# facebookresearch/rela

Hardware: AMD Instinct MI355X
Metric: env-steps/s (Ape-X Atari 84x84x4, actor tick + learner grad-step) (higher is better)
Workload: dtype f32 (f32 operands as 3 exact bf16 parts on bf16 MFMA; f32-accurate); 1 GPU; Ape-X DQN 80x80 envs/GPU, actor+learner on one MI355X, replay 2^20, B=512, A=18, n=3; device-resident static frames; parallelism=single

## Files before the change

### include/rela_amd.h

```cpp
#ifndef RELA_AMD_H
#define RELA_AMD_H

#include <stdint.h>

#ifdef __cplusplus
extern "C" {
#endif

#define RELA_OK 0
#define RELA_EINVAL (-1)
#define RELA_ENODEV (-2)
#define RELA_ENOMEM (-3)
#define RELA_ESTATE (-4)
#define RELA_ESCAN (-5)
#define RELA_EWOULDBLOCK (-6)

const char* rela_last_error(void);
int rela_abi_version(void);

int rela_stream_create(void** out, int device);
void rela_stream_destroy(void* stream, int device);
int rela_stream_synchronize(void* stream, int device);
int rela_stream_wait_stream(void* waiter, void* signaler, int device);
int rela_memcpy_h2d_async(void* dst_dev, const void* src_host, int64_t bytes, void* stream, int device);
// ... 129 lines not shown
                                  void* stream);
int rela_ffnet_debug_fc_stamps(const rela_ffnet* net, int n, const uint8_t* a3_records, unsigned long long* out_host,
                               void* stream);
int64_t rela_ffnet_workspace_bytes(const rela_ffnet* net, int n);
enum { RELA_WS_NOT_WRITTEN = 0, RELA_WS_F32 = 1, RELA_WS_SPLIT_BF16 = 2, RELA_WS_SPLIT3 = 3 };
typedef struct {
  int64_t a1, a2, a3, h, ha, gx, fc_part, rec2, rec3;
  int32_t precision, trunk, fc, fc_slices, fc_per;
  int32_t a1_format, a2_format, a3_format;
  int32_t a3_records, x_in_gx;
} rela_debug_workspace_view;
int rela_ffnet_debug_workspace(const rela_ffnet* net, int n, rela_debug_workspace_view* view);
int rela_ffnet_debug_forward_store_frames(const rela_ffnet* net, int n, const uint8_t* s_dev, const float* legal_dev,
                                          float* q_dev, void* workspace_dev, int64_t workspace_bytes, void* rows_dev,
                                          int first, int ring, int* copied, void* stream);

int rela_ffnet_forward(const rela_ffnet* net, int n, const uint8_t* s_dev, const float* legal_dev,
                       float* q_dev, void* workspace_dev, int64_t workspace_bytes, void* stream);

int rela_apex_act_from_q(int n, int num_action, int group_rows, const float* q_dev,
                         const float* legal_dev, const float* eps_dev, uint64_t rng_seed,
                         uint64_t rng_offset, int64_t* action_dev, void* stream);

int rela_apex_td_from_q(int n, int num_action, int group_rows, const float* q_dev,
                        const float* q_next_online_dev,
                        const float* q_next_target_dev, const float* next_legal_dev,
                        const int64_t* action_dev, const float* reward_dev,
                        const float* bootstrap_dev, float gamma_n, float* td_err_dev,
                        float* priority_dev, void* stream);

// ... 267 lines not shown
```

### rela_amd/_capi.py

```python
import ctypes as C
import os

import torch

PKG = os.path.dirname(os.path.abspath(__file__))
LIB_PATH = os.path.join(PKG, "librela_amd.so")

if not os.path.exists(LIB_PATH):
    raise ImportError(
        "rela_amd: %s is missing -- the HIP extension has not been built (python -m rela_amd.build). "
        "There is no CPU fallback for this path." % LIB_PATH)

lib = C.CDLL(LIB_PATH)

OK, EINVAL, ENODEV, ENOMEM, ESTATE, ESCAN, EWOULDBLOCK = 0, -1, -2, -3, -4, -5, -6

vp, i32, i64, u64, f32, f64 = C.c_void_p, C.c_int, C.c_int64, C.c_uint64, C.c_float, C.c_double
P = C.POINTER


class ReplayState(C.Structure):
    _fields_ = [("head", C.c_int32), ("tail", C.c_int32), ("size", C.c_int32), ("safe_size", C.c_int32),
                ("ring", C.c_int32), ("n_sampled", C.c_int32), ("num_add", C.c_int64), ("sum", C.c_double),
                ("dev_error", C.c_int32), ("pad", C.c_int32)]
# ... 143 lines not shown
_sig("rela_ffnet_num_action", i32, [vp])
_sig("rela_ffnet_version", C.c_uint64, [vp])
_sig("rela_ffnet_set_precision", i32, [vp, i32])
_sig("rela_ffnet_precision", i32, [vp])
_sig("rela_ffnet_debug_conv12_stamps", i32, [vp, i32, vp, vp, vp])
_sig("rela_ffnet_debug_fc_stamps", i32, [vp, i32, vp, vp, vp])
_sig("rela_ffnet_debug_conv3_stamps", i32, [vp, i32, vp, vp, vp])
_sig("rela_ffnet_debug_conv12_records", i32, [vp, i32, vp, vp, vp, vp, vp, vp])
_sig("rela_ffnet_debug_layout", i32, [vp, i32, P(C.c_char_p), P(i64), P(i32), vp])
_sig("rela_lstmnet_debug_layout", i32, [vp, i32, P(C.c_char_p), P(i64), P(i32), vp])
_sig("rela_lstmnet_set_precision", i32, [vp, i32])
_sig("rela_lstmnet_precision", i32, [vp])
_sig("rela_ffnet_workspace_bytes", i64, [vp, i32])
_sig("rela_ffnet_debug_workspace", i32, [vp, i32, P(DebugWorkspaceView)])
_sig("rela_ffnet_debug_forward_store_frames", i32, [vp, i32, vp, vp, vp, vp, i64, vp, i32, i32, P(i32), vp])
_sig("rela_lstmnet_debug_workspace", i32, [vp, i32, P(DebugWorkspaceView)])
_sig("rela_ffnet_forward", i32, [vp, i32, vp, vp, vp, vp, i64, vp])
_sig("rela_lstmnet_create", i32, [P(vp), i32, i32])
_sig("rela_lstmnet_destroy", None, [vp])
_sig("rela_lstmnet_load", i32, [vp, P(LSTMNetParams), i32, vp])
_sig("rela_lstmnet_num_action", i32, [vp])
_sig("rela_lstmnet_version", C.c_uint64, [vp])
_sig("rela_lstmnet_workspace_bytes", i64, [vp, i32])
_sig("rela_lstmnet_step", i32, [vp, i32, vp, vp, vp, vp, vp, vp, vp, vp, vp, i64, vp])
_sig("rela_apex_act_from_q", i32, [i32, i32, i32, vp, vp, vp, u64, u64, vp, vp])
_sig("rela_apex_td_from_q", i32, [i32, i32, i32, vp, vp, vp, vp, vp, vp, vp, f32, vp, vp, vp])
_sig("rela_apex_actor_create", i32, [P(vp), i32, i32, i32, i32, f32, vp, u64, i32])
_sig("rela_apex_actor_destroy", None, [vp])
_sig("rela_apex_actor_obs_slot", vp, [vp])
_sig("rela_apex_actor_plane_stage", vp, [vp])
# ... 122 lines not shown
```

### rela_amd/csrc/actor.hip

```cpp
#include <cmath>

#include "actor_shard.h"
#include "ffnet_layout.h"

using namespace rela_amd;

struct rela_apex_actor : ActorShardBase {
  float gamma = 0.f, gamma_n = 0.f;
  uint64_t seed = 0;
  float* prio = nullptr;
  void* ws = nullptr;
  int64_t ws_bytes = 0;
  int64_t key_tick = -1;
};

namespace {
constexpr int kTickWin = 64;
}

extern "C" int rela_apex_actor_create(rela_apex_actor** out, int rows, int group_rows, int num_action, int multi_step,
                                      float gamma, rela_replay* replay, uint64_t seed, int device) {
  RELA_CHECK(out && rows >= 1 && group_rows >= 1 && rows % group_rows == 0 && num_action >= 1 && num_action <= 31 &&
                 multi_step >= 1,
             RELA_EINVAL, "rela_apex_actor_create: bad arguments (rows=%d group=%d A=%d n=%d)", rows, group_rows,
// ... 38 lines not shown
extern "C" int rela_apex_actor_set_screen_input(rela_apex_actor* a, int height, int width) {
  return shard_set_screen_input(a, height, width, 3, "rela_apex_actor_set_screen_input");
}
extern "C" int rela_apex_actor_set_screen_input_indexed(rela_apex_actor* a, int height, int width) {
  return shard_set_screen_input(a, height, width, 1, "rela_apex_actor_set_screen_input_indexed");
}
extern "C" void* rela_apex_actor_palette_stage(rela_apex_actor* a) { return a ? a->palettes : nullptr; }
extern "C" void* rela_apex_actor_screen_stage(rela_apex_actor* a) { return a ? a->screens : nullptr; }
extern "C" int rela_apex_actor_screens_to_stacks(rela_apex_actor* a, const uint8_t* restart_host, void* stream_) {
  return shard_screens_to_stacks(a, restart_host, (hipStream_t)stream_, "rela_apex_actor_screens_to_stacks");
}
extern "C" int rela_apex_actor_set_reuse(rela_apex_actor* a, int on) {
  return shard_set_reuse(a, on, "rela_apex_actor_set_reuse");
}
extern "C" int rela_apex_actor_set_fused_insert(rela_apex_actor* a, int on) {
  RELA_CHECK(a && (on == 0 || on == 1), RELA_EINVAL, "rela_apex_actor_set_fused_insert: 0 (off) or 1 (on)");
  a->fused_insert = on != 0;
  return RELA_OK;
}
extern "C" int rela_apex_actor_set_value_rescale(rela_apex_actor* a, float eps) {
  return shard_set_value_rescale(a, eps, "rela_apex_actor_set_value_rescale");
}
extern "C" int rela_apex_actor_set_dedup(rela_apex_actor* a, int units_per_stack) {
  const int rc = shard_set_dedup_common(a, units_per_stack, 0, "rela_apex_actor_set_dedup");
  if (rc == RELA_OK) a->tick_seq.assign(kTickWin, 0);
  return rc;
}
extern "C" float* rela_apex_actor_eps_dev(rela_apex_actor* a) { return a ? a->eps : nullptr; }
extern "C" float* rela_apex_actor_legal_dev(rela_apex_actor* a) { return a ? a->legal : nullptr; }
extern "C" int64_t rela_apex_actor_num_act(const rela_apex_actor* a) { return a ? a->num_act.load() : 0; }
extern "C" const float* rela_apex_actor_last_q_dev(const rela_apex_actor* a) {
  return a ? a->q_hist + (size_t)(a->q_slot < 0 ? 0 : a->q_slot) * a->R * a->A : nullptr;
// ... 96 lines not shown
  if (a->fused_insert && a->dd_ups == 0 && piece == a->R && ffnet_forward_stores_frames(target, a->R)) {
    rc = rela_replay_begin_add(a->replay, a->R, nonblocking, &fused_slot);
    if (rc == RELA_EWOULDBLOCK) fused_slot = -1;
    else if (rc != RELA_OK) return rc;
  }
  if (fused_slot >= 0) {
    void* base = nullptr;
    int rows_ring = 0;
    int64_t row_bytes = 0;
    rc = rela_replay_direct_rows(a->replay, fused_slot, a->R, 1, &base, &rows_ring, &row_bytes, s);
    if (rc == RELA_OK && row_bytes != kObs) {
      set_last_error("rela_apex_actor_post_step: the replay's next_obs rows have %lld bytes, a frame stack %lld",
                     (long long)row_bytes, (long long)kObs);
      rc = RELA_EINVAL;
    }
    if (rc == RELA_OK)
      rc = ffnet_forward_store_frames(target, a->R, obs_n, legal_n, a->q + 3 * QA, a->ws, a->ws_bytes, s,
                                      FrameRows{static_cast<uint8_t*>(base), fused_slot, rows_ring}, &fused_copied);
  } else {
    rc = rela_ffnet_forward(target, a->R, obs_n, legal_n, a->q + 3 * QA, a->ws, a->ws_bytes, s);
  }
  const int64_t* act_t = a->act + (size_t)first * a->R;
  if (rc == RELA_OK)
    rc = td_from_q(a->R, a->A, a->K, q_online_t, q_online_n, a->q + 3 * QA, legal_n, act_t, a->out_r, a->out_b, a->gamma_n,
                   a->vr_eps, nullptr, a->prio, s);
  if (rc != RELA_OK) {
    if (fused_slot >= 0) (void)rela_replay_abort_add(a->replay, fused_slot, a->R);
    return rc;
  }
  const void* rows[10] = {obs_t, obs_n, eps_t, eps_n, legal_t, legal_n, act_t, a->out_r, a->out_t, a->out_b};
  if (a->dd_ups > 0) {
    rows[0] = a->ref_hist + (size_t)first * a->R * a->dd_ups;
    rows[1] = a->ref_hist + (size_t)last * a->R * a->dd_ups;
  }
  const int64_t stack_rb = a->dd_ups > 0 ? (int64_t)sizeof(int32_t) * a->dd_ups : kObs;
  const int64_t rb[10] = {stack_rb, stack_rb, 4, 4, 4 * a->A, 4 * a->A, 8, 4, 1, 4};
  int dropped = dd_drop ? 1 : 0;
  for (int off = 0; off < a->R && !dd_drop; off += piece) {
    const int cnt = a->R - off < piece ? a->R - off : piece;
    const void* prow[10];
    for (int f = 0; f < 10; ++f) prow[f] = static_cast<const uint8_t*>(rows[f]) + (int64_t)off * rb[f];
    int slot = fused_slot;
    if (fused_slot >= 0) {
      if (fused_copied) prow[1] = nullptr;
    } else {
      rc = rela_replay_begin_add(a->replay, cnt, nonblocking, &slot);
      if (rc == RELA_EWOULDBLOCK) {
        dropped = 1;
        continue;
      }
      if (rc != RELA_OK) break;
    }
    if (a->dd_ups > 0) (void)rela_replay_set_block_min_unit(a->replay, slot, cnt, dd_min_seq);
    rc = rela_replay_write_rows(a->replay, slot, 0, cnt, prow, s);
    if (rc == RELA_OK) rc = rela_replay_commit_add_grouped(a->replay, slot, cnt, a->K, a->prio + off, s);
    if (rc != RELA_OK) {
      (void)rela_replay_abort_add(a->replay, slot, cnt);
      break;
    }
// ... 8 lines not shown
```

### rela_amd/csrc/actor_shard.h

```cpp
#pragma once
#include <atomic>
#include <vector>

#include "common.h"
#include "dedup_refs.h"

namespace rela_amd {

constexpr int64_t kObs = 4 * 84 * 84;
constexpr int64_t kPlane = 84 * 84;

struct ActorShardBase {
  int device = 0;
  int R = 0, K = 0, A = 0, n = 0;
  rela_replay* replay = nullptr;
  uint64_t act_calls = 0;
  std::atomic<int64_t> num_act{0};
  int head = 0, count = 0, cur = -1;
  uint8_t* obs = nullptr;
  int64_t* act = nullptr;
  float* rew = nullptr;
  uint8_t* term = nullptr;
  float* eps = nullptr;
  float* legal = nullptr;
  float* eps_hist = nullptr;
  float* legal_hist = nullptr;
  float* q = nullptr;
  float* q_hist = nullptr;
  float *out_r = nullptr, *out_b = nullptr;
  uint8_t* out_t = nullptr;
  std::vector<const void*> qh_net;
  std::vector<uint64_t> qh_version;
  int q_slot = -1;
  int reuse_mode = 1;
  bool fused_insert = true;
  float vr_eps = 0.f;
  uint8_t* restart = nullptr;
  uint8_t* fresh_planes = nullptr;
  uint8_t* screens = nullptr;
  uint8_t* palettes = nullptr;
  uint8_t* screen_prev = nullptr;
  int scr_h = 0, scr_w = 0;
  int dd_ups = 0;
  int64_t dd_cap = 0;
  int32_t* ref_hist = nullptr;
  std::vector<uint8_t> refs_valid;
  std::vector<int64_t> tick_seq;
  int64_t tick = 0;
};

// ... 210 lines not shown
```

### rela_amd/csrc/conv12_s3.h

```cpp
#pragma once
#include <hip/hip_runtime.h>

#include "gemm_s3.h"

namespace rela_amd {
namespace s3 {

typedef int i32x4 __attribute__((ext_vector_type(4)));
typedef uint32_t u32x4_a4 __attribute__((ext_vector_type(4), aligned(4)));
#ifndef C12_ABLATE
#define C12_ABLATE 0
#endif

constexpr bool kNoCopyOut = C12_ABLATE == 1, kNoStage = C12_ABLATE == 2, kNoEpi1 = C12_ABLATE == 3, kNoEpi2 = C12_ABLATE == 4,
               kNoConv1 = C12_ABLATE == 5, kNoConv2 = C12_ABLATE == 6;

struct Conv12S {
  static constexpr int kT = 256;
  static constexpr int GW = 21, NPIX = GW * GW, PLANE_ELEMS = 84 * 84, IN_ELEMS = 4 * PLANE_ELEMS;
  static constexpr int PLANE1 = 7168;
  static constexpr int T1_BYTES = 4 * PLANE1;
  static constexpr int Q = 13, RQ = 261;
  static constexpr int T2_BYTES = 20 * RQ * 16;
  static constexpr int OROW = 400;
  static constexpr int C2TILES = 5, C2PIX = C2TILES * 16;
  static constexpr int O_BYTES = C2PIX * OROW;
  static constexpr int RING_S = 5;
  static constexpr int PATCH_UNITS = 16 * 12, SLOT_BYTES = 202 * 16;
  static constexpr int RING = T1_BYTES + T2_BYTES + O_BYTES;
  static constexpr int LDS_TOTAL = RING + RING_S * SLOT_BYTES;
  static_assert(LDS_TOTAL <= 160 * 1024, "LDS budget");
  static_assert(RING_S >= 1 && RING_S <= 16, "one slot per lane of a tile's column");
  static constexpr int OV16 = C2PIX * 24, OIT = (OV16 + kT - 1) / kT;
  static constexpr int UNITS = 4 * GW * 6, UIT = (UNITS + kT - 1) / kT;
  static constexpr int KS2 = 16;
  static constexpr int tap2(int ks) {
    const int c = ks >> 2, j = ks & 3;
    const int dh = j >> 1, dw = (j ^ (j >> 1)) & 1;
    return (((c >> 1) + 2 * dh) << 2) | ((c & 1) + 2 * dw);
  }
  static constexpr int koff2(int ks) { return ((tap2(ks) >> 2) * RQ + (tap2(ks) & 3) * Q) * 16; }
};

template <bool A1OUT, bool COPY>
__device__ __forceinline__ void conv12_s3_body(const uint8_t* __restrict__ in, const uint4* __restrict__ W1d,
                                               const float* __restrict__ scale1, const float* __restrict__ bias1q,
                                               const uint4* __restrict__ B2, const float* __restrict__ bias2,
                                               uint8_t* __restrict__ out, float* __restrict__ a1_out, int N,
                                               uint8_t* __restrict__ copy_dst, int copy_first, int copy_ring) {
  using F = Conv12S;
  extern __shared__ __attribute__((aligned(16))) uint8_t smem_c12[];
  uint8_t* t1 = smem_c12;
  uint8_t* t2 = t1 + F::T1_BYTES;
  uint8_t* otile = t2 + F::T2_BYTES;
  const int tid = threadIdx.x, lane = tid & 63, li = lane & 15, g = lane >> 4;
  const int wave = __builtin_amdgcn_readfirstlane(tid >> 6);
  const int bid = blockIdx.x, nblk = gridDim.x;
  int n = bid;
  if (n >= N) return;

  const int ct1 = wave & 1, rg1 = wave >> 1;
  bf16x8 w2[F::KS2][3];
  {
    const uint4* bp = B2 + (size_t)wave * 3 * 64 + lane;
// ... 33 lines not shown
    ugoff[j] = (uint32_t)(pl * F::PLANE_ELEMS + 4 * Y * 84 + 4 * X0);
    uloff[j] = (uint32_t)(pl * F::PLANE1 + (Y * F::GW + X0) * 16);
  }
  auto g_load4 = [&](int fr, int j) __attribute__((always_inline)) {
    const uint8_t* fb = in + (size_t)fr * F::IN_ELEMS;
#pragma unroll
    for (int r = 0; r < 4; ++r) sq[j][r] = *reinterpret_cast<const u32x4_a4*>(fb + (size_t)ugoff[j] + r * 84);
  };
  auto copy_row = [&](int fr) __attribute__((always_inline)) -> uint8_t* {
    int sl = copy_first + fr;
    if (sl >= copy_ring) sl -= copy_ring;
    return copy_dst + (size_t)sl * F::IN_ELEMS;
  };
  auto g_copy4 = [&](uint8_t* cb, int j, int r) __attribute__((always_inline)) {
    *reinterpret_cast<u32x4_a4*>(cb + (size_t)ugoff[j] + r * 84) = sq[j][r];
  };
  auto s_store4 = [&](int j, int k) __attribute__((always_inline)) {
    *reinterpret_cast<uint4*>(t1 + uloff[j] + k * 16) = make_uint4(sq[j][0][k] ^ 0x80808080u, sq[j][1][k] ^ 0x80808080u,
                                                                   sq[j][2][k] ^ 0x80808080u, sq[j][3][k] ^ 0x80808080u);
  };

  int prev = -1;
  static_assert(F::OIT == 8, "eight named chunk registers (an array indexed inside the hooks stays in scratch)");
  uint4 oc0, oc1, oc2, oc3, oc4, oc5, oc6, oc7;
  auto oc_at = [&](auto jt) -> uint4& {
    constexpr int j = decltype(jt)::value;
    if constexpr (j == 0) return oc0;
    else if constexpr (j == 1) return oc1;
    else if constexpr (j == 2) return oc2;
    else if constexpr (j == 3) return oc3;
// ... 82 lines not shown
      *reinterpret_cast<uint2*>(rec + 64) = p1;
      *reinterpret_cast<uint2*>(rec + 128) = p2;
      if constexpr (A1OUT) {
        uint8_t* ab = reinterpret_cast<uint8_t*>(a1_out + ((size_t)n * 400 + rt * 16) * 32);
        *reinterpret_cast<f32x4*>(ab + (size_t)a1lane) = v;
      }
    }
  };

#pragma unroll
  for (int j = 0; j < F::UIT; ++j) g_load4(n, j);
#pragma unroll
  for (int j = 0; j < F::UIT; ++j)
#pragma unroll
    for (int k = 0; k < 4; ++k) s_store4(j, k);
  if constexpr (COPY) {
    uint8_t* cb = copy_row(n);
#pragma unroll
    for (int j = 0; j < F::UIT; ++j)
#pragma unroll
      for (int r = 0; r < 4; ++r) g_copy4(cb, j, r);
  }
  __syncthreads();

  auto copy_hook = [&](auto idx_tag) {
    constexpr int IDX = decltype(idx_tag)::value;
    if constexpr (!kNoCopyOut && IDX < 2 * F::OIT) {
      if constexpr (IDX % 2 == 0) o_read(IC<IDX / 2>{});
      else o_write(IC<IDX / 2>{});
    }
  };
  auto no_hook = [](auto) {};
  static_assert(2 * F::OIT <= 20, "copy-out slots inside conv1's first pass");

  uint32_t xbh[F::C2TILES];
#pragma unroll
  for (int t = 0; t < F::C2TILES; ++t) {
    const int m = t * 16 + li;
    const int oy = m / 9, ox = m - oy * 9;
    xbh[t] = (uint32_t)((2 * oy * F::RQ + 2 * ox * F::Q + g) * 16);
  }
  uint32_t o2dst[F::C2TILES];
#pragma unroll
  for (int t = 0; t < F::C2TILES; ++t) o2dst[t] = (uint32_t)(F::T1_BYTES + F::T2_BYTES + (t * 16 + li) * F::OROW + ch2 * 2);
  uint32_t psrc, pdst;
  {
    const int t = min(tid, F::PATCH_UNITS - 1);
// ... 39 lines not shown
      f32x4 v = acc + accs;
#pragma unroll
      for (int r = 0; r < 4; ++r) v[r] = v[r] > 0.f ? v[r] : 0.f;
      uint2 p0, p1, p2;
      split3_4(v, p0, p1, p2);
      uint8_t* rec = out + (size_t)(first + sl * nblk) * (81 * 384) + (F::C2PIX * 384 + ch2 * 2);
      *reinterpret_cast<uint2*>(rec) = p0;
      *reinterpret_cast<uint2*>(rec + 128) = p1;
      *reinterpret_cast<uint2*>(rec + 256) = p2;
    }
  };
  int filled = 0;
  for (; n < N; n += nblk) {
    const int nn = (n + nblk < N) ? n + nblk : n;
    uint8_t* cbn = nullptr;
    if constexpr (COPY) cbn = copy_row(nn);
    pin_weights();
    conv1_pass(IC<0>{}, IC<5>{}, copy_hook);
    conv1_pass(IC<5>{}, IC<4>{}, no_hook);
    conv1_pass(IC<9>{}, IC<4>{}, no_hook);
    if constexpr (kNoEpi1) asm volatile("" ::"v"(sc1), "v"(bv1));
    __syncthreads();
    {
      constexpr int TOT = F::C2TILES * F::KS2, D = 3;
      const uint4 patch = *reinterpret_cast<const uint4*>(t2 + psrc);
      uint4 xr[D][3];
      auto a_issue = [&](auto idx_tag, int slot) {
        constexpr int IDX = decltype(idx_tag)::value, T = IDX / F::KS2, KS = IDX - T * F::KS2;
        const uint8_t* ap = t2 + xbh[T] + F::koff2(KS);
        xr[slot][0] = *reinterpret_cast<const uint4*>(ap);
        xr[slot][1] = *reinterpret_cast<const uint4*>(ap + 64);
        xr[slot][2] = *reinterpret_cast<const uint4*>(ap + 128);
      };
      static_for<D>([&](auto i) { a_issue(i, decltype(i)::value); });
      __builtin_amdgcn_sched_barrier(0);
// ... 6 lines not shown
          accs = __builtin_amdgcn_mfma_f32_16x16x32_bf16(w2[KS][2], x0, accs, 0, 0, 0);
          accs = __builtin_amdgcn_mfma_f32_16x16x32_bf16(w2[KS][0], x2, accs, 0, 0, 0);
          accs = __builtin_amdgcn_mfma_f32_16x16x32_bf16(w2[KS][1], x1, accs, 0, 0, 0);
          accs = __builtin_amdgcn_mfma_f32_16x16x32_bf16(w2[KS][1], x0, accs, 0, 0, 0);
          accs = __builtin_amdgcn_mfma_f32_16x16x32_bf16(w2[KS][0], x1, accs, 0, 0, 0);
          acc = __builtin_amdgcn_mfma_f32_16x16x32_bf16(w2[KS][0], x0, acc, 0, 0, 0);
        } else {
          asm volatile("" ::"v"(x0), "v"(x1), "v"(x2));
        }
        if constexpr (IDX + D < TOT) a_issue(IC<IDX + D>{}, SLOT);
        if constexpr (IDX == 2) *reinterpret_cast<uint4*>(smem_c12 + pdst + filled * F::SLOT_BYTES) = patch;
        static_for<4 * F::UIT>([&](auto jj) {
          constexpr int JJ = decltype(jj)::value;
          if constexpr (JJ < F::UIT && IDX == 1 + 12 * JJ && !kNoStage) g_load4(nn, JJ);
          if constexpr (IDX == TOT / 2 + 4 * JJ && !kNoStage) s_store4(JJ >> 2, JJ & 3);
          if constexpr (COPY && IDX == TOT / 2 + 4 * JJ && !kNoStage) g_copy4(cbn, JJ >> 2, JJ & 3);
        });
        if constexpr (KS == F::KS2 - 1 && kNoEpi2) asm volatile("" ::"v"(acc), "v"(accs));
        if constexpr (KS == F::KS2 - 1 && !kNoEpi2) {
          f32x4 v = acc + accs;
#pragma unroll
          for (int r = 0; r < 4; ++r) v[r] = v[r] > 0.f ? v[r] : 0.f;
          uint2 p0, p1, p2;
          split3_4(v, p0, p1, p2);
          uint8_t* rec = smem_c12 + o2dst[T];
          *reinterpret_cast<uint2*>(rec) = p0;
          *reinterpret_cast<uint2*>(rec + 128) = p1;
          *reinterpret_cast<uint2*>(rec + 256) = p2;
          acc = bv2, accs = f32x4{0.f, 0.f, 0.f, 0.f};
        }
        __builtin_amdgcn_sched_barrier(0);
// ... 8 lines not shown
  }
  {
    uint4* dst = reinterpret_cast<uint4*>(out + (size_t)prev * (81 * 384));
    for (int i = tid; i < F::OV16; i += F::kT) {
      const int px = i / 24, u = i - px * 24;
      dst[i] = *reinterpret_cast<const uint4*>(otile + px * F::OROW + u * 16);
    }
  }
}

template <bool A1OUT>
__global__ __launch_bounds__(256, 1) void conv12_s3(const uint8_t* __restrict__ in, const uint4* __restrict__ W1d,
                                                    const float* __restrict__ scale1, const float* __restrict__ bias1q,
                                                    const uint4* __restrict__ B2, const float* __restrict__ bias2,
                                                    uint8_t* __restrict__ out, float* __restrict__ a1_out, int N) {
  conv12_s3_body<A1OUT, false>(in, W1d, scale1, bias1q, B2, bias2, out, a1_out, N, nullptr, 0, 0);
}
__global__ __launch_bounds__(256, 1) void conv12_s3_copy(const uint8_t* __restrict__ in, const uint4* __restrict__ W1d,
                                                         const float* __restrict__ scale1, const float* __restrict__ bias1q,
                                                         const uint4* __restrict__ B2, const float* __restrict__ bias2,
                                                         uint8_t* __restrict__ out, int N, uint8_t* __restrict__ copy_dst,
                                                         int copy_first, int copy_ring) {
  conv12_s3_body<false, true>(in, W1d, scale1, bias1q, B2, bias2, out, nullptr, N, copy_dst, copy_first, copy_ring);
}

inline void launch_conv12(const uint8_t* frames, const uint4* W1d, const float* s1q, const float* b1q, const uint4* B2e,
                          const float* b2, uint8_t* rec2, float* a1, int N, hipStream_t s, int blocks) {
  const auto kernel = a1 ? conv12_s3<true> : conv12_s3<false>;
  hipLaunchKernelGGL(kernel, dim3(blocks), dim3(Conv12S::kT), Conv12S::LDS_TOTAL, s, frames, W1d, s1q, b1q, B2e, b2, rec2, a1, N);
}
inline void launch_conv12_copy(const uint8_t* frames, const uint4* W1d, const float* s1q, const float* b1q, const uint4* B2e,
                               const float* b2, uint8_t* rec2, int N, hipStream_t s, int blocks, uint8_t* copy_dst,
                               int copy_first, int copy_ring) {
  hipLaunchKernelGGL(conv12_s3_copy, dim3(blocks), dim3(Conv12S::kT), Conv12S::LDS_TOTAL, s, frames, W1d, s1q, b1q, B2e, b2, rec2,
                     N, copy_dst, copy_first, copy_ring);
}
inline int opt_in_lds_conv12() {
  for (const void* k : {reinterpret_cast<const void*>(&conv12_s3<false>), reinterpret_cast<const void*>(&conv12_s3<true>),
                        reinterpret_cast<const void*>(&conv12_s3_copy)})
    RELA_HIP(hipFuncSetAttribute(k, hipFuncAttributeMaxDynamicSharedMemorySize, Conv12S::LDS_TOTAL));
  return RELA_OK;
}

}
}
```

### rela_amd/csrc/ffnet.hip

```cpp
#include "common.h"
#include "gemm_bf16s.h"
#include "gemm_f32emu.h"
#include "gemm_s3.h"
#include "conv_img_s3.h"
#include "conv12_s3.h"
#include "ffnet_layout.h"
#include "ffnet_plan.h"
#include "conv_f32.h"
#include "gemm_f32.h"
#include "conv12_i8.h"
#include "fc_bf16s.h"
#include "heads_duel.h"
#include "param_layout.h"
#include "prof.h"
#define RELA_WEIGHT_PACK_KERNEL
#include "weight_pack.h"

namespace rela_amd {

struct FFNetDev {
  uint4* B1 = nullptr;
  float* b1 = nullptr;
  float *B2 = nullptr, *b2 = nullptr;
  float *B3 = nullptr, *b3 = nullptr;
// ... 50 lines not shown
struct TrunkLabels {
  const char *conv1, *conv2, *conv3, *conv12;
};
struct TrunkOpts {
  bool keep_f32 = false;
  bool leave_a3_records = false;
  const FrameRows* store_frames = nullptr;
};
void launch_trunk(const FFNetDev& d, TrunkKind kind, int N, const uint8_t* s_dev, float* a1, float* a2, float* a3,
                  uint8_t* rec2, uint8_t* rec3, const TrunkOpts& o, const TrunkLabels& l, hipStream_t s) {
  switch (kind) {
    case kTrunkS3: {
      {
        ProfScope prof(l.conv12, s);
        note_launch("conv12_s3");
        if (o.store_frames) {
          note_launch("conv12_s3_copy");
          s3::launch_conv12_copy(s_dev, d.W1d, d.s1q, d.b1q, d.B2e, d.b2, rec2, N, s, persistent_blocks(N), o.store_frames->base,
                                 o.store_frames->first, o.store_frames->ring);
        } else {
          s3::launch_conv12(s_dev, d.W1d, d.s1q, d.b1q, d.B2e, d.b2, rec2, o.keep_f32 ? a1 : nullptr, N, s, persistent_blocks(N));
        }
      }
      ProfScope prof(l.conv3, s);
      note_launch("conv3_img_s3");
      s3::launch_conv3_img(rec2, d.B3e, d.b3, rec3, N, s, persistent_blocks(N));
      break;
    }
    case kTrunkBf16: {
      {
        ProfScope prof(l.conv12, s);
// ... 340 lines not shown
  return rela_amd::ffnet_forward_mode(n, N, s_dev, legal_dev, q_dev, ws, ws_bytes, stream_, kModeNet);
}

int rela_amd::ffnet_forward_mode(const rela_ffnet* n, int N, const uint8_t* s_dev, const float* legal_dev, float* q_dev,
                                 void* ws, int64_t ws_bytes, void* stream_, int mode, int rows_limit) {
  return forward_impl(n, N, s_dev, legal_dev, q_dev, ws, ws_bytes, stream_, mode, rows_limit, nullptr, nullptr);
}

bool rela_amd::ffnet_forward_stores_frames(const rela_ffnet* n, int N) {
  return n && N >= 1 && plan_ffnet_forward(kModeNet, n->precision, N, n->max_rows).trunk == kTrunkS3;
}
int rela_amd::ffnet_forward_store_frames(const rela_ffnet* n, int N, const uint8_t* s_dev, const float* legal_dev, float* q_dev,
                                         void* ws, int64_t ws_bytes, void* stream_, const FrameRows& rows, int* copied) {
  RELA_CHECK(copied && rows.base && ((uintptr_t)rows.base & 3) == 0 && rows.first >= 0 && rows.first < rows.ring && N <= rows.ring,
             RELA_EINVAL, "ffnet_forward_store_frames: bad frame rows (first %d, ring %d, %d frames)", rows.first, rows.ring, N);
  return forward_impl(n, N, s_dev, legal_dev, q_dev, ws, ws_bytes, stream_, kModeNet, -1, &rows, copied);
}

extern "C" int rela_ffnet_debug_forward_store_frames(const rela_ffnet* n, int N, const uint8_t* s_dev, const float* legal_dev,
                                                     float* q_dev, void* ws, int64_t ws_bytes, void* rows_dev, int first,
                                                     int ring, int* copied, void* stream_) {
  return rela_amd::ffnet_forward_store_frames(n, N, s_dev, legal_dev, q_dev, ws, ws_bytes, stream_,
                                              FrameRows{static_cast<uint8_t*>(rows_dev), first, ring}, copied);
}

static int forward_impl(const rela_ffnet* n, int N, const uint8_t* s_dev, const float* legal_dev, float* q_dev, void* ws,
                        int64_t ws_bytes, void* stream_, int mode, int rows_limit, const FrameRows* store, int* copied) {
  if (copied) *copied = 0;
  RELA_CHECK(n && n->loaded, RELA_ESTATE, "rela_ffnet_forward: parameters were never loaded");
  const int max_rows = rows_limit < 0 ? n->max_rows : rows_limit;
  RELA_CHECK(N >= 1 && s_dev && legal_dev && q_dev && ws, RELA_EINVAL, "rela_ffnet_forward: bad arguments");
  RELA_CHECK(ws_bytes >= rela_ffnet_workspace_bytes(n, N), RELA_EINVAL,
             "rela_ffnet_forward: workspace of %lld bytes is too small for batch %d", (long long)ws_bytes, N);
  RELA_CHECK(((uintptr_t)s_dev & 15) == 0 && ((uintptr_t)ws & 15) == 0, RELA_EINVAL,
             "rela_ffnet_forward: s_dev and workspace must be 16-byte aligned");
  RELA_CHECK(max_rows <= 0 || N <= max_rows, RELA_EINVAL,
             "rela_ffnet_forward: batch %d on a net whose owner declared at most %d rows", N, max_rows);
  hipStream_t s = (hipStream_t)stream_;
// ... 7 lines not shown
    if (int rc = pack_one(kLayouts[kLayBfT].kind, n->bft_src, nullptr, n->d.BfT, 0, 0, kLayouts[kLayBfT].elements, s)) return rc;
    n->packed |= lay_bit(kLayBfT);
    missing = 0;
  }
  RELA_CHECK(missing == 0, RELA_ESTATE,
             "rela_ffnet_forward: %d rows in mode %d read layouts (bits 0x%x) the net's last load did not pack (row limit %d)", N,
             plan.precision, missing, n->max_rows);

  uint8_t* rec2 = static_cast<uint8_t*>(ws) + ws_records_offset(N);
  uint8_t* rec3 = rec2 + (int64_t)N * kRec2Bytes;
  TrunkOpts opts;
  opts.keep_f32 = plan.keep_f32;
  opts.leave_a3_records = !plan.unsplit_a3;
  if (store && plan.trunk == kTrunkS3 && !plan.keep_f32) {
    opts.store_frames = store;
    *copied = 1;
  }
  launch_trunk(d, plan.trunk, N, s_dev, w.a1, w.a2, w.a3, rec2, rec3, opts, {names[0], names[1], names[2], name12}, s);

  float* const part = fc_part_ptr(ws, w.ha, N);
  switch (plan.fc) {
    case kFcBf16: {
      ProfScope prof(names[3], s);
      launch_fc_bf16s(recs(w.a3), d.Bff, d.bf, w.h, N, s);
      break;
    }
    case kFcBf16SplitK:
      launch_fc_bf16_splitk(recs(w.a3), d.Bff, d.bf, part, w.h, N, names[3], s);
      break;
    case kFcS3:
    case kFcS3SplitK: {
// ... 289 lines not shown
```

### rela_amd/csrc/ffnet_layout.h

```cpp
#pragma once
#include <hip/hip_runtime.h>

#include <cstdint>

namespace rela_amd {

constexpr int64_t kA1 = 400 * 32, kA2 = 81 * 64, kA3 = 49 * 64, kH = 512, kHA = 32;
constexpr int64_t kWsFloatsPerSample = kA1 + kA2 + kA3 + kH + kHA;
constexpr int64_t kRec2Bytes = 81 * 384, kRec3Bytes = 49 * 384;

struct FFNetWs {
  float *a1, *a2, *a3, *h, *ha;
};

inline FFNetWs ffnet_ws(void* ws, int N) {
  FFNetWs w;
  w.a1 = static_cast<float*>(ws);
  w.a2 = w.a1 + kA1 * N;
  w.a3 = w.a2 + kA2 * N;
  w.h = w.a3 + kA3 * N;
  w.ha = w.h + kH * N;
  return w;
}

// ... 16 lines not shown
};
}

#include "../../include/rela_amd.h"
namespace rela_amd {
int ffnet_load_extra(rela_ffnet* n, const rela_ffnet_params* p, void* stream, const ExtraPacks& extra);
int lstmnet_load_extra(rela_lstmnet* n, const rela_lstmnet_params* p, void* stream, const ExtraPacks& extra);
void ffnet_label_as_learner(rela_ffnet* n);
void ffnet_set_max_rows(rela_ffnet* n, int rows);
int ffnet_forward_mode(const rela_ffnet* n, int N, const uint8_t* s_dev, const float* legal_dev, float* q_dev, void* ws,
                       int64_t ws_bytes, void* stream, int mode, int rows_limit = -1);
constexpr int64_t kFrameBytes = 4 * 84 * 84;
struct FrameRows {
  uint8_t* base;
  int first, ring;
};
bool ffnet_forward_stores_frames(const rela_ffnet* n, int N);
int ffnet_forward_store_frames(const rela_ffnet* n, int N, const uint8_t* s_dev, const float* legal_dev, float* q_dev, void* ws,
                               int64_t ws_bytes, void* stream, const FrameRows& rows, int* copied);
bool ffnet_learner_forward_ok(const rela_ffnet* on, const rela_ffnet* tg, int B);
int ffnet_learner_forward(const rela_ffnet* on, const rela_ffnet* tg, int B, const uint8_t* s_obs, const uint8_t* s_next,
                          const float* legal, const float* nlegal, float* q_on, float* q_no, float* q_nt, void* ws_on,
                          void* ws_tg, int64_t ws_bytes, hipStream_t s);
int ffnet_learner_unsplit(int B, void* ws_on, hipStream_t s);

int lstmnet_trunk(const rela_lstmnet* n, int N, const uint8_t* s_dev, float* a1, float* a2, float* a3, hipStream_t s,
                  const char* const* names, bool fast = false, bool* a3_records = nullptr, uint8_t* s3_scratch = nullptr,
                  bool keep_f32 = true);
int64_t gate_x3_packed_bytes();
int pack_gate_x3(const float* w_ih_dev, void* dst, bool permuted, hipStream_t s);
// ... 8 lines not shown
```

### rela_amd/engine.py

```python
import ctypes as C

import torch

from . import _capi as capi
from .replay import OBS_BYTES


class _NetHandle:

    _PREFIX = _PARAMS = KEYS = None

    def _fn(self, what):
        return getattr(capi.lib, "rela_%s_%s" % (self._PREFIX, what))

    def __init__(self, num_action, device="cuda:0"):
        self.device = torch.device(device)
        self.num_action = num_action
        h = C.c_void_p()
        capi.check(self._fn("create")(C.byref(h), num_action, self.device.index or 0), "rela_%s_create" % self._PREFIX)
        self.h = h

    def load_state_dict(self, sd, prefix=""):
        p = self._PARAMS()
        keep = []
# ... 80 lines not shown
    @property
    def num_act(self):
        return capi.lib.rela_apex_actor_num_act(self.h)

    @property
    def q(self):
        return dev_view(capi.lib.rela_apex_actor_last_q_dev(self.h), (1, self._rows, self._A), torch.float32, self.device)

    def set_value_rescale(self, eps):
        capi.check(capi.lib.rela_apex_actor_set_value_rescale(self.h, float(eps)), "rela_apex_actor_set_value_rescale")

    def set_reuse(self, on):
        capi.check(capi.lib.rela_apex_actor_set_reuse(self.h, int(on)), "rela_apex_actor_set_reuse")

    def set_fused_insert(self, on):
        capi.check(capi.lib.rela_apex_actor_set_fused_insert(self.h, int(bool(on))), "rela_apex_actor_set_fused_insert")

    def next_obs_slot(self):
        ptr = capi.lib.rela_apex_actor_obs_slot(self.h)
        return dev_view(ptr, (self.R, 4, 84, 84), torch.uint8, self.device)

    def act(self, online):
        out = C.c_void_p()
        capi.check(capi.lib.rela_apex_actor_act(self.h, online.h, None, None, None, None, C.byref(out), self._stream()),
                   "rela_apex_actor_act")
        return dev_view(out.value, (self.R,), torch.int64, self.device)

    def post_step(self, reward, terminal, online, target, nonblocking=False):
        ins = C.c_int(0)
        self._keep = (reward, terminal)
        rc = capi.lib.rela_apex_actor_post_step(self.h, C.c_void_p(reward.data_ptr()), C.c_void_p(terminal.data_ptr()),
# ... 79 lines not shown
```

Measured before the change: 3.691 million env-steps/s.

## Fuse obs frame-stack replay insert into target conv12 forward kernel

The fused replay insert now covers the current observation stack as well as the next observation. The conv12 kernel gains a second copy stream whose global loads and stores are interleaved at fixed slots inside the conv1/conv2 passes, so the obs row no longer goes through the separate replay add copy. This is on by default (mode 2). It adds register pressure and extra memory traffic inside an already tuned persistent kernel, which could slow the conv itself.

```diff
diff --git a/include/rela_amd.h b/include/rela_amd.h
--- a/include/rela_amd.h
+++ b/include/rela_amd.h
@@ -167,6 +167,10 @@
 int rela_ffnet_debug_forward_store_frames(const rela_ffnet* net, int n, const uint8_t* s_dev, const float* legal_dev,
                                           float* q_dev, void* workspace_dev, int64_t workspace_bytes, void* rows_dev,
                                           int first, int ring, int* copied, void* stream);
+int rela_ffnet_debug_forward_store_frames2(const rela_ffnet* net, int n, const uint8_t* s_dev, const float* legal_dev,
+                                           float* q_dev, void* workspace_dev, int64_t workspace_bytes, void* rows_dev,
+                                           int first, int ring, const uint8_t* s2_dev, void* rows2_dev, int first2,
+                                           int* copied, void* stream);
 
 int rela_ffnet_forward(const rela_ffnet* net, int n, const uint8_t* s_dev, const float* legal_dev,
                        float* q_dev, void* workspace_dev, int64_t workspace_bytes, void* stream);
diff --git a/rela_amd/_capi.py b/rela_amd/_capi.py
--- a/rela_amd/_capi.py
+++ b/rela_amd/_capi.py
@@ -181,6 +181,7 @@
 _sig("rela_ffnet_workspace_bytes", i64, [vp, i32])
 _sig("rela_ffnet_debug_workspace", i32, [vp, i32, P(DebugWorkspaceView)])
 _sig("rela_ffnet_debug_forward_store_frames", i32, [vp, i32, vp, vp, vp, vp, i64, vp, i32, i32, P(i32), vp])
+_sig("rela_ffnet_debug_forward_store_frames2", i32, [vp, i32, vp, vp, vp, vp, i64, vp, i32, i32, vp, vp, i32, P(i32), vp])
 _sig("rela_lstmnet_debug_workspace", i32, [vp, i32, P(DebugWorkspaceView)])
 _sig("rela_ffnet_forward", i32, [vp, i32, vp, vp, vp, vp, i64, vp])
 _sig("rela_lstmnet_create", i32, [P(vp), i32, i32])
diff --git a/rela_amd/csrc/actor.hip b/rela_amd/csrc/actor.hip
--- a/rela_amd/csrc/actor.hip
+++ b/rela_amd/csrc/actor.hip
@@ -76,8 +76,8 @@
   return shard_set_reuse(a, on, "rela_apex_actor_set_reuse");
 }
 extern "C" int rela_apex_actor_set_fused_insert(rela_apex_actor* a, int on) {
-  RELA_CHECK(a && (on == 0 || on == 1), RELA_EINVAL, "rela_apex_actor_set_fused_insert: 0 (off) or 1 (on)");
-  a->fused_insert = on != 0;
+  RELA_CHECK(a && on >= 0 && on <= 2, RELA_EINVAL, "rela_apex_actor_set_fused_insert: 0 (off), 1 (next_obs) or 2 (next_obs and obs)");
+  a->fused_insert = on;
   return RELA_OK;
 }
 extern "C" int rela_apex_actor_set_value_rescale(rela_apex_actor* a, float eps) {
@@ -204,9 +204,22 @@
                      (long long)row_bytes, (long long)kObs);
       rc = RELA_EINVAL;
     }
+    FrameRows fr{static_cast<uint8_t*>(base), fused_slot, rows_ring};
+    if (rc == RELA_OK && a->fused_insert == 2) {
+      void* base0 = nullptr;
+      int ring0 = 0;
+      rc = rela_replay_direct_rows(a->replay, fused_slot, a->R, 0, &base0, &ring0, &row_bytes, s);
+      if (rc == RELA_OK && (row_bytes != kObs || ring0 != rows_ring)) {
+        set_last_error("rela_apex_actor_post_step: the replay's obs rows have %lld bytes in a ring of %d, a frame stack %lld in %d",
+                       (long long)row_bytes, ring0, (long long)kObs, rows_ring);
+        rc = RELA_EINVAL;
+      }
+      fr.src2 = obs_t;
+      fr.base2 = static_cast<uint8_t*>(base0);
+      fr.first2 = fused_slot;
+    }
     if (rc == RELA_OK)
-      rc = ffnet_forward_store_frames(target, a->R, obs_n, legal_n, a->q + 3 * QA, a->ws, a->ws_bytes, s,
-                                      FrameRows{static_cast<uint8_t*>(base), fused_slot, rows_ring}, &fused_copied);
+      rc = ffnet_forward_store_frames(target, a->R, obs_n, legal_n, a->q + 3 * QA, a->ws, a->ws_bytes, s, fr, &fused_copied);
   } else {
     rc = rela_ffnet_forward(target, a->R, obs_n, legal_n, a->q + 3 * QA, a->ws, a->ws_bytes, s);
   }
@@ -232,7 +245,8 @@
     for (int f = 0; f < 10; ++f) prow[f] = static_cast<const uint8_t*>(rows[f]) + (int64_t)off * rb[f];
     int slot = fused_slot;
     if (fused_slot >= 0) {
-      if (fused_copied) prow[1] = nullptr;
+      if (fused_copied >= 1) prow[1] = nullptr;
+      if (fused_copied >= 2) prow[0] = nullptr;
     } else {
       rc = rela_replay_begin_add(a->replay, cnt, nonblocking, &slot);
       if (rc == RELA_EWOULDBLOCK) {
diff --git a/rela_amd/csrc/actor_shard.h b/rela_amd/csrc/actor_shard.h
--- a/rela_amd/csrc/actor_shard.h
+++ b/rela_amd/csrc/actor_shard.h
@@ -33,7 +33,7 @@
   std::vector<uint64_t> qh_version;
   int q_slot = -1;
   int reuse_mode = 1;
-  bool fused_insert = true;
+  int fused_insert = 2;
   float vr_eps = 0.f;
   uint8_t* restart = nullptr;
   uint8_t* fresh_planes = nullptr;
diff --git a/rela_amd/csrc/conv12_s3.h b/rela_amd/csrc/conv12_s3.h
--- a/rela_amd/csrc/conv12_s3.h
+++ b/rela_amd/csrc/conv12_s3.h
@@ -14,6 +14,7 @@
 
 constexpr bool kNoCopyOut = C12_ABLATE == 1, kNoStage = C12_ABLATE == 2, kNoEpi1 = C12_ABLATE == 3, kNoEpi2 = C12_ABLATE == 4,
                kNoConv1 = C12_ABLATE == 5, kNoConv2 = C12_ABLATE == 6;
+constexpr bool kNoPtStore = C12_ABLATE == 7, kNoPtLoad = C12_ABLATE == 8;
 
 struct Conv12S {
   static constexpr int kT = 256;
@@ -42,12 +43,14 @@
   static constexpr int koff2(int ks) { return ((tap2(ks) >> 2) * RQ + (tap2(ks) & 3) * Q) * 16; }
 };
 
-template <bool A1OUT, bool COPY>
+template <bool A1OUT, int COPY>
 __device__ __forceinline__ void conv12_s3_body(const uint8_t* __restrict__ in, const uint4* __restrict__ W1d,
                                                const float* __restrict__ scale1, const float* __restrict__ bias1q,
                                                const uint4* __restrict__ B2, const float* __restrict__ bias2,
                                                uint8_t* __restrict__ out, float* __restrict__ a1_out, int N,
-                                               uint8_t* __restrict__ copy_dst, int copy_first, int copy_ring) {
+                                               uint8_t* __restrict__ copy_dst, int copy_first, int copy_ring,
+                                               const uint8_t* __restrict__ in2, uint8_t* __restrict__ copy2_dst,
+                                               int copy2_first) {
   using F = Conv12S;
   extern __shared__ __attribute__((aligned(16))) uint8_t smem_c12[];
   uint8_t* t1 = smem_c12;
@@ -111,6 +114,19 @@
   };
   auto g_copy4 = [&](uint8_t* cb, int j, int r) __attribute__((always_inline)) {
     *reinterpret_cast<u32x4_a4*>(cb + (size_t)ugoff[j] + r * 84) = sq[j][r];
+  };
+  u32x4_a4 pt[4] = {};
+  uint8_t* cb2 = nullptr;
+  auto pt_load = [&](auto p_tag) __attribute__((always_inline)) {
+    constexpr int P = decltype(p_tag)::value;
+    const uint8_t* fb = in2 + (size_t)n * F::IN_ELEMS;
+    if constexpr (!kNoPtLoad) pt[P & 3] = *reinterpret_cast<const u32x4_a4*>(fb + (size_t)ugoff[P >> 2] + (P & 3) * 84);
+  };
+  auto pt_store = [&](auto p_tag) __attribute__((always_inline)) {
+    constexpr int P = decltype(p_tag)::value;
+    const u32x4_a4 v = pt[P & 3];
+    if constexpr (!kNoPtStore) *reinterpret_cast<u32x4_a4*>(cb2 + (size_t)ugoff[P >> 2] + (P & 3) * 84) = v;
+    else asm volatile("" ::"v"(v));
   };
   auto s_store4 = [&](int j, int k) __attribute__((always_inline)) {
     *reinterpret_cast<uint4*>(t1 + uloff[j] + k * 16) = make_uint4(sq[j][0][k] ^ 0x80808080u, sq[j][1][k] ^ 0x80808080u,
@@ -223,7 +239,7 @@
   for (int j = 0; j < F::UIT; ++j)
 #pragma unroll
     for (int k = 0; k < 4; ++k) s_store4(j, k);
-  if constexpr (COPY) {
+  if constexpr (COPY != 0) {
     uint8_t* cb = copy_row(n);
 #pragma unroll
     for (int j = 0; j < F::UIT; ++j)
@@ -239,7 +255,11 @@
       else o_write(IC<IDX / 2>{});
     }
   };
-  auto no_hook = [](auto) {};
+  auto pass_hook = [&](auto idx_tag) {
+    constexpr int IDX = decltype(idx_tag)::value;
+    if constexpr (COPY == 2 && IDX >= 20 && (IDX - 20) % 8 == 0 && !kNoStage) pt_load(IC<(IDX - 20) / 8>{});
+  };
+  constexpr int kPtStore[8] = {4, 8, 12, 16, 27, 31, 35, 39}, kPtLoad[8] = {-1, -1, -1, -1, 6, 10, 15, 18};
   static_assert(2 * F::OIT <= 20, "copy-out slots inside conv1's first pass");
 
   uint32_t xbh[F::C2TILES];
@@ -309,11 +329,16 @@
   for (; n < N; n += nblk) {
     const int nn = (n + nblk < N) ? n + nblk : n;
     uint8_t* cbn = nullptr;
-    if constexpr (COPY) cbn = copy_row(nn);
+    if constexpr (COPY != 0) cbn = copy_row(nn);
+    if constexpr (COPY == 2) {
+      int sl = copy2_first + n;
+      if (sl >= copy_ring) sl -= copy_ring;
+      cb2 = copy2_dst + (size_t)sl * F::IN_ELEMS;
+    }
     pin_weights();
     conv1_pass(IC<0>{}, IC<5>{}, copy_hook);
-    conv1_pass(IC<5>{}, IC<4>{}, no_hook);
-    conv1_pass(IC<9>{}, IC<4>{}, no_hook);
+    conv1_pass(IC<5>{}, IC<4>{}, pass_hook);
+    conv1_pass(IC<9>{}, IC<4>{}, pass_hook);
     if constexpr (kNoEpi1) asm volatile("" ::"v"(sc1), "v"(bv1));
     __syncthreads();
     {
@@ -350,7 +375,9 @@
           constexpr int JJ = decltype(jj)::value;
           if constexpr (JJ < F::UIT && IDX == 1 + 12 * JJ && !kNoStage) g_load4(nn, JJ);
           if constexpr (IDX == TOT / 2 + 4 * JJ && !kNoStage) s_store4(JJ >> 2, JJ & 3);
-          if constexpr (COPY && IDX == TOT / 2 + 4 * JJ && !kNoStage) g_copy4(cbn, JJ >> 2, JJ & 3);
+          if constexpr (COPY != 0 && IDX == TOT / 2 + 4 * JJ && !kNoStage) g_copy4(cbn, JJ >> 2, JJ & 3);
+          if constexpr (COPY == 2 && IDX == kPtStore[JJ] && !kNoStage) pt_store(IC<JJ>{});
+          if constexpr (COPY == 2 && IDX == kPtLoad[JJ] && !kNoStage) pt_load(IC<JJ>{});
         });
         if constexpr (KS == F::KS2 - 1 && kNoEpi2) asm volatile("" ::"v"(acc), "v"(accs));
         if constexpr (KS == F::KS2 - 1 && !kNoEpi2) {
@@ -389,14 +416,24 @@
                                                     const float* __restrict__ scale1, const float* __restrict__ bias1q,
                                                     const uint4* __restrict__ B2, const float* __restrict__ bias2,
                                                     uint8_t* __restrict__ out, float* __restrict__ a1_out, int N) {
-  conv12_s3_body<A1OUT, false>(in, W1d, scale1, bias1q, B2, bias2, out, a1_out, N, nullptr, 0, 0);
+  conv12_s3_body<A1OUT, 0>(in, W1d, scale1, bias1q, B2, bias2, out, a1_out, N, nullptr, 0, 0, nullptr, nullptr, 0);
 }
 __global__ __launch_bounds__(256, 1) void conv12_s3_copy(const uint8_t* __restrict__ in, const uint4* __restrict__ W1d,
                                                          const float* __restrict__ scale1, const float* __restrict__ bias1q,
                                                          const uint4* __restrict__ B2, const float* __restrict__ bias2,
                                                          uint8_t* __restrict__ out, int N, uint8_t* __restrict__ copy_dst,
                                                          int copy_first, int copy_ring) {
-  conv12_s3_body<false, true>(in, W1d, scale1, bias1q, B2, bias2, out, nullptr, N, copy_dst, copy_first, copy_ring);
+  conv12_s3_body<false, 1>(in, W1d, scale1, bias1q, B2, bias2, out, nullptr, N, copy_dst, copy_first, copy_ring, nullptr, nullptr,
+                           0);
+}
+__global__ __launch_bounds__(256, 1) void conv12_s3_copies2(const uint8_t* __restrict__ in, const uint4* __restrict__ W1d,
+                                                            const float* __restrict__ scale1, const float* __restrict__ bias1q,
+                                                            const uint4* __restrict__ B2, const float* __restrict__ bias2,
+                                                            uint8_t* __restrict__ out, int N, uint8_t* __restrict__ copy_dst,
+                                                            int copy_first, int copy_ring, const uint8_t* __restrict__ in2,
+                                                            uint8_t* __restrict__ copy2_dst, int copy2_first) {
+  conv12_s3_body<false, 2>(in, W1d, scale1, bias1q, B2, bias2, out, nullptr, N, copy_dst, copy_first, copy_ring, in2, copy2_dst,
+                           copy2_first);
 }
 
 inline void launch_conv12(const uint8_t* frames, const uint4* W1d, const float* s1q, const float* b1q, const uint4* B2e,
@@ -410,9 +447,15 @@
   hipLaunchKernelGGL(conv12_s3_copy, dim3(blocks), dim3(Conv12S::kT), Conv12S::LDS_TOTAL, s, frames, W1d, s1q, b1q, B2e, b2, rec2,
                      N, copy_dst, copy_first, copy_ring);
 }
+inline void launch_conv12_copy2(const uint8_t* frames, const uint4* W1d, const float* s1q, const float* b1q, const uint4* B2e,
+                                const float* b2, uint8_t* rec2, int N, hipStream_t s, int blocks, uint8_t* copy_dst,
+                                int copy_first, int copy_ring, const uint8_t* frames2, uint8_t* copy2_dst, int copy2_first) {
+  hipLaunchKernelGGL(conv12_s3_copies2, dim3(blocks), dim3(Conv12S::kT), Conv12S::LDS_TOTAL, s, frames, W1d, s1q, b1q, B2e, b2, rec2,
+                     N, copy_dst, copy_first, copy_ring, frames2, copy2_dst, copy2_first);
+}
 inline int opt_in_lds_conv12() {
   for (const void* k : {reinterpret_cast<const void*>(&conv12_s3<false>), reinterpret_cast<const void*>(&conv12_s3<true>),
-                        reinterpret_cast<const void*>(&conv12_s3_copy)})
+                        reinterpret_cast<const void*>(&conv12_s3_copy), reinterpret_cast<const void*>(&conv12_s3_copies2)})
     RELA_HIP(hipFuncSetAttribute(k, hipFuncAttributeMaxDynamicSharedMemorySize, Conv12S::LDS_TOTAL));
   return RELA_OK;
 }
diff --git a/rela_amd/csrc/ffnet.hip b/rela_amd/csrc/ffnet.hip
--- a/rela_amd/csrc/ffnet.hip
+++ b/rela_amd/csrc/ffnet.hip
@@ -88,7 +88,12 @@
       {
         ProfScope prof(l.conv12, s);
         note_launch("conv12_s3");
-        if (o.store_frames) {
+        if (o.store_frames && o.store_frames->src2) {
+          note_launch("conv12_s3_copy2");
+          s3::launch_conv12_copy2(s_dev, d.W1d, d.s1q, d.b1q, d.B2e, d.b2, rec2, N, s, persistent_blocks(N), o.store_frames->base,
+                                  o.store_frames->first, o.store_frames->ring, o.store_frames->src2, o.store_frames->base2,
+                                  o.store_frames->first2);
+        } else if (o.store_frames) {
           note_launch("conv12_s3_copy");
           s3::launch_conv12_copy(s_dev, d.W1d, d.s1q, d.b1q, d.B2e, d.b2, rec2, N, s, persistent_blocks(N), o.store_frames->base,
                                  o.store_frames->first, o.store_frames->ring);
@@ -459,6 +464,13 @@
                                          void* ws, int64_t ws_bytes, void* stream_, const FrameRows& rows, int* copied) {
   RELA_CHECK(copied && rows.base && ((uintptr_t)rows.base & 3) == 0 && rows.first >= 0 && rows.first < rows.ring && N <= rows.ring,
              RELA_EINVAL, "ffnet_forward_store_frames: bad frame rows (first %d, ring %d, %d frames)", rows.first, rows.ring, N);
+  if (rows.src2) {
+    const uint8_t *b1 = rows.base, *b2 = rows.base2;
+    const int64_t len = (int64_t)rows.ring * kFrameBytes;
+    RELA_CHECK(b2 && (((uintptr_t)b2 | (uintptr_t)rows.src2) & 3) == 0 && rows.first2 >= 0 && rows.first2 < rows.ring &&
+                   (b2 + len <= b1 || b1 + len <= b2),
+               RELA_EINVAL, "ffnet_forward_store_frames: bad second frame rows (first %d, ring %d)", rows.first2, rows.ring);
+  }
   return forward_impl(n, N, s_dev, legal_dev, q_dev, ws, ws_bytes, stream_, kModeNet, -1, &rows, copied);
 }
 
@@ -467,6 +479,15 @@
                                                      int ring, int* copied, void* stream_) {
   return rela_amd::ffnet_forward_store_frames(n, N, s_dev, legal_dev, q_dev, ws, ws_bytes, stream_,
                                               FrameRows{static_cast<uint8_t*>(rows_dev), first, ring}, copied);
+}
+extern "C" int rela_ffnet_debug_forward_store_frames2(const rela_ffnet* n, int N, const uint8_t* s_dev, const float* legal_dev,
+                                                      float* q_dev, void* ws, int64_t ws_bytes, void* rows_dev, int first,
+                                                      int ring, const uint8_t* s2_dev, void* rows2_dev, int first2, int* copied,
+                                                      void* stream_) {
+  RELA_CHECK(s2_dev && rows2_dev, RELA_EINVAL, "rela_ffnet_debug_forward_store_frames2: no second source or destination");
+  return rela_amd::ffnet_forward_store_frames(
+      n, N, s_dev, legal_dev, q_dev, ws, ws_bytes, stream_,
+      FrameRows{static_cast<uint8_t*>(rows_dev), first, ring, s2_dev, static_cast<uint8_t*>(rows2_dev), first2}, copied);
 }
 
 static int forward_impl(const rela_ffnet* n, int N, const uint8_t* s_dev, const float* legal_dev, float* q_dev, void* ws,
@@ -504,7 +525,7 @@
   opts.leave_a3_records = !plan.unsplit_a3;
   if (store && plan.trunk == kTrunkS3 && !plan.keep_f32) {
     opts.store_frames = store;
-    *copied = 1;
+    *copied = store->src2 ? 2 : 1;
   }
   launch_trunk(d, plan.trunk, N, s_dev, w.a1, w.a2, w.a3, rec2, rec3, opts, {names[0], names[1], names[2], name12}, s);
 
diff --git a/rela_amd/csrc/ffnet_layout.h b/rela_amd/csrc/ffnet_layout.h
--- a/rela_amd/csrc/ffnet_layout.h
+++ b/rela_amd/csrc/ffnet_layout.h
@@ -54,6 +54,9 @@
 struct FrameRows {
   uint8_t* base;
   int first, ring;
+  const uint8_t* src2 = nullptr;
+  uint8_t* base2 = nullptr;
+  int first2 = 0;
 };
 bool ffnet_forward_stores_frames(const rela_ffnet* n, int N);
 int ffnet_forward_store_frames(const rela_ffnet* n, int N, const uint8_t* s_dev, const float* legal_dev, float* q_dev, void* ws,
diff --git a/rela_amd/engine.py b/rela_amd/engine.py
--- a/rela_amd/engine.py
+++ b/rela_amd/engine.py
@@ -118,7 +118,7 @@
         capi.check(capi.lib.rela_apex_actor_set_reuse(self.h, int(on)), "rela_apex_actor_set_reuse")
 
     def set_fused_insert(self, on):
-        capi.check(capi.lib.rela_apex_actor_set_fused_insert(self.h, int(bool(on))), "rela_apex_actor_set_fused_insert")
+        capi.check(capi.lib.rela_apex_actor_set_fused_insert(self.h, int(on)), "rela_apex_actor_set_fused_insert")
 
     def next_obs_slot(self):
         ptr = capi.lib.rela_apex_actor_obs_slot(self.h)
```

After: 3.811 million env-steps/s (median of 6 runs). 1.03x the previous value.
